# UltronAI/Depth-VO-Feat

Measured on AMD Instinct MI355X. Metric: KITTI 256x832 stereo-seq samples/sec fwd+bwd, higher is better.
Workload: dtype f32

## Files before the change

### depth-vo-feat_amd/csrc/conv_pipe.h

```cpp
#pragma once
#include "dvf_common.h"

namespace dvfp {

#ifdef DVF_TUNING
#define DVF_STAMP(a, var) do { if ((a).stamps) asm volatile("s_memtime %0\n\ts_waitcnt lgkmcnt(0)" : "=s"(var) :: "memory"); } while (0)
#define DVF_STAMP_RT(a, var) do { if ((a).stamps) asm volatile("s_memrealtime %0\n\ts_waitcnt lgkmcnt(0)" : "=s"(var) :: "memory"); } while (0)
#define DVF_STAMPS_ON 1
#else
#define DVF_STAMP(a, var) do { } while (0)
#define DVF_STAMP_RT(a, var) do { } while (0)
#define DVF_STAMPS_ON 0
#endif

typedef float f32x16 __attribute__((ext_vector_type(16)));
typedef __attribute__((address_space(3))) void lds_void_t;

__device__ __forceinline__ __amdgpu_buffer_rsrc_t tensor_rsrc(const void *p) {
    const uint64_t v = reinterpret_cast<uint64_t>(p);
    const unsigned lo = __builtin_amdgcn_readfirstlane((unsigned)v), hi = __builtin_amdgcn_readfirstlane((unsigned)(v >> 32));
    return __builtin_amdgcn_make_buffer_rsrc(reinterpret_cast<void *>(((uint64_t)hi << 32) | lo), 0, 0x7FFFFFF0, 0x00020000);
}
constexpr unsigned OOB = 0x80000000u;
__device__ __forceinline__ float bload(__amdgpu_buffer_rsrc_t r, unsigned voff, unsigned soff) {
// ... 13 lines not shown
    int segC[DVF_MAX_SEGS];
    int nseg;
    const float *wp;
    const float *bias;
    float *out;
    int M, N, IH, IW, OH, OW;
    int OS, IS, ncls;
    PClass cls[4];
    int act;
    float alpha, beta;
    int KS, NCH, out_mode, NG;
    int64_t ws_slice;
    int lsw, lsh, TGX, TGY, BW, BH, BN, tilesX, tilesY;
    int x4;
    int blk;
    int SLmax, PSRmax, NST;
    int dbg;
    unsigned long long *stamps;
    const float *mask;
};

__host__ __device__ inline int pipe_row_stride(int RSu, int SW, int SH, int IS) {
    if (SH == 1 || SW >= 32 || (SW % IS) != 0) return RSu;
    const int mod = 32 / IS, want = (SW / IS) % mod;
    const int padded = RSu + ((want - RSu % mod) + mod) % mod;
    return (padded * 8 <= RSu * 9) ? padded : RSu;
}

struct PipeGeo { int PH, PW, PWH, RS, PSR, NPI, XA; };
__host__ __device__ inline PipeGeo pipe_geo(int BH, int BW, int BN, int IS, int TA, int TB, int SW, int SH, int x4 = 0, int bx = 0) {
// ... 9 lines not shown
            int padded = rs;
            while (((padded * IS) & 31) != ((SW * IS) & 31) && padded < rs + 32) padded += 4;
            if (((padded * IS) & 31) == ((SW * IS) & 31) && padded * 8 <= rs * 9) rs = padded;
        }
        g.RS = rs;
        g.PSR = (BN * g.PH * g.RS + 255) & ~255;
        g.NPI = g.PSR >> 8;
        return g;
    }
    g.RS = pipe_row_stride(IS == 2 ? 2 * g.PWH : g.PW, SW, SH, IS);
    g.PSR = (BN * g.PH * g.RS + 63) & ~63;
    g.NPI = g.PSR >> 6;
    return g;
}

template <int V> struct fvec;
template <> struct fvec<1> { typedef float type; };
template <> struct fvec<2> { typedef float type __attribute__((ext_vector_type(2))); };
template <> struct fvec<4> { typedef float type __attribute__((ext_vector_type(4))); };

constexpr int PIPE_THREADS = 384;
constexpr int PIPE_THREADS_4P = 512;
constexpr int PIPE_MAXNPI = 32;

template <int MT, int NT, int WM, int CKH, int TBU, int BLK = 0>
__global__ __launch_bounds__(PIPE_THREADS_4P) void conv_pipe_kernel(const PipeArgs a) {
    constexpr int CK = 2 * CKH, VW = CKH >= 4 ? 4 : CKH, CPG = CKH / VW, MTW = MT * WM;
    constexpr int UNITF = TBU * MTW * 64 * VW;
    typedef typename fvec<VW>::type avec;
    extern __shared__ __attribute__((aligned(16))) float smem[];
    const int stage_floats = a.SLmax + CK * a.PSRmax;
    const int tid = threadIdx.x, lane = tid & 63, nl = lane & 31, kh = lane >> 5;
    const int wave = __builtin_amdgcn_readfirstlane(tid >> 6);
    const int zper = gridDim.z / a.ncls;
    const int zc = blockIdx.z / zper, zr = blockIdx.z - zc * zper;
    const int ng = zr / a.KS, ks = zr - ng * a.KS;
    const PClass c = a.cls[zc];
    const int tX = blockIdx.x % a.tilesX, tY = blockIdx.x / a.tilesX;
    const int oy0 = tY * a.BH, ox0 = tX * a.BW, n0 = ng * a.BN;
    if (oy0 >= c.OHc || ox0 >= c.OWc) return;
    const int mb = blockIdx.y;
    const int SW = 1 << a.lsw, SH = 1 << a.lsh;
// ... 176 lines not shown
    const int NU = c.NTG * CPG;
    int opy[NT], opx[NT], opn[NT];
    int bj[NT][VW];
    const int pxl = nl & (SW - 1), pyl = (nl >> a.lsw) & (SH - 1), pnl = nl >> (a.lsw + a.lsh);
#pragma unroll
    for (int i = 0; i < NT; ++i) {
        const int q = wn * NT + i, tx = q % a.TGX, tyn = q / a.TGX, ty = tyn % a.TGY, tn = tyn / a.TGY;
        const int SN = 32 >> (a.lsw + a.lsh);
        opy[i] = ty * SH + pyl;
        opx[i] = tx * SW + pxl;
        opn[i] = tn * SN + pnl;
        const int bbase = kh * PSR + (opn[i] * geo.PH + opy[i] * a.IS) * RS + (a.x4 ? geo.XA + opx[i] * a.IS : opx[i]);
#pragma unroll
        for (int j = 0; j < VW; ++j) bj[i][j] = bbase + j * 2 * PSR;
    }
    f32x16 acc[MT][NT];
    f32x16 asum[BLK ? MT : 1][BLK ? NT : 1];
#pragma unroll
    for (int m = 0; m < MT; ++m)
#pragma unroll
        for (int i = 0; i < NT; ++i)
#pragma unroll
            for (int r = 0; r < 16; ++r) {
                acc[m][i][r] = 0.f;
                if constexpr (BLK) asum[m][i][r] = 0.f;
            }

    auto consume = [&](int st, auto isc, auto tbec) {
        constexpr int IS = decltype(isc)::value, TBE = decltype(tbec)::value;
        const float *wl = smem + st * stage_floats;
        const float *patch = wl + a.SLmax;
        const float *ap = wl + (wm * MT) * 64 * VW + lane * VW;
        avec af[2][MT];
        float bf[2][TBE][NT][VW];
        int lta = 0, lcpg = 0, lk = 0;
        auto load_bj = [&](auto bufc, auto jc) {
            constexpr int buf = decltype(bufc)::value, j = decltype(jc)::value;
            const float *prow0 = patch + (lta * RS + lcpg * (2 * VW) * PSR);
#pragma unroll
            for (int i = 0; i < NT; ++i) {
                const float *prow = prow0 + bj[i][j];
// ... 21 lines not shown
        };
        auto advance = [&]() {
            ++lk;
            const bool wrap = (lcpg + 1 == CPG);
            lcpg = wrap ? 0 : lcpg + 1;
            lta += wrap ? 1 : 0;
        };
        auto mma_j = [&](auto bufc, auto tpc, auto uc, auto jc) {
            constexpr int buf = decltype(bufc)::value, tp = decltype(tpc)::value, u = decltype(uc)::value, j = decltype(jc)::value;
#pragma unroll
            for (int m = 0; m < MT; ++m) {
                float av;
                if constexpr (VW == 1) av = af[tp][m]; else av = af[tp][m][j];
#pragma unroll
                for (int i = 0; i < NT; ++i)
                    acc[m][i] = __builtin_amdgcn_mfma_f32_32x32x2f32(av, bf[buf][u][i][j], acc[m][i], 0, 0, 0);
            }
        };
        using B0 = std::integral_constant<int, 0>;
        using B1 = std::integral_constant<int, 1>;
        auto step = [&](auto bufc, auto nbufc, auto pbc, auto uc) {
            constexpr int u = decltype(uc)::value, tp = (decltype(pbc)::value + u) & 1;
            using TP = std::integral_constant<int, tp>;
            mma_j(bufc, TP{}, uc, std::integral_constant<int, 0>{});
            __builtin_amdgcn_sched_barrier(0);
            if constexpr (u + 1 < TBE) load_a(std::integral_constant<int, tp ^ 1>{}, lk - 1, std::integral_constant<int, u + 1>{});
            else load_a(std::integral_constant<int, tp ^ 1>{}, lk, std::integral_constant<int, 0>{});
            if constexpr (u == 0) load_bj(nbufc, std::integral_constant<int, 0>{});
            __builtin_amdgcn_sched_barrier(0);
            if constexpr (VW > 1) {
                mma_j(bufc, TP{}, uc, std::integral_constant<int, 1>{});
// ... 19 lines not shown
            if constexpr (TBE > 4) step(bufc, nbufc, pbc, std::integral_constant<int, 4>{});
            if constexpr (TBE > 5) step(bufc, nbufc, pbc, std::integral_constant<int, 5>{});
            if constexpr (TBE > 6) step(bufc, nbufc, pbc, std::integral_constant<int, 6>{});
            advance();
        };
        load_b(B0{});
        load_a(B0{}, 0, std::integral_constant<int, 0>{});
        advance();
        __builtin_amdgcn_sched_barrier(0);
        for (int k = 0; k < NU; k += 2) {
            unit(B0{}, B1{}, std::integral_constant<int, 0>{});
            if (k + 1 < NU) unit(B1{}, B0{}, std::integral_constant<int, TBE & 1>{});
        }
    };

    unsigned long long t_loop0 = 0, t_loop1 = 0, tb0 = 0, tb1 = 0, w_bar = 0;
    DVF_STAMP(a, t_loop0);
    if (!DVF_DBG(a, 8)) {
        int st = 0, since = 0;
        for (int g = g_begin; g < g_end; ++g) {
            DVF_STAMP(a, tb0);
            __syncthreads();
            DVF_STAMP(a, tb1);
            w_bar += tb1 - tb0;
            if (!DVF_DBG(a, 4)) {
                using TBfull = std::integral_constant<int, TBU>;
                using TBless = std::integral_constant<int, (TBU > 1 ? TBU - 1 : 1)>;
                if (a.IS == 2 && !a.x4) consume(st, std::integral_constant<int, 2>{}, TBfull{});
                else if (TBU > 1 && c.TB == TBU - 1 && !DVF_DBG(a, 64)) consume(st, std::integral_constant<int, 1>{}, TBless{});
                else consume(st, std::integral_constant<int, 1>{}, TBfull{});
            }
            if constexpr (BLK) {
                if (++since == a.blk) {
                    since = 0;
#pragma unroll
                    for (int m = 0; m < MT; ++m)
#pragma unroll
                        for (int i = 0; i < NT; ++i) {
                            asum[m][i] += acc[m][i];
#pragma unroll
                            for (int r = 0; r < 16; ++r) acc[m][i][r] = 0.f;
                        }
                }
            }
            st = (st + 1 == a.NST) ? 0 : st + 1;
        }
    }
    if constexpr (BLK) {
#pragma unroll
        for (int m = 0; m < MT; ++m)
#pragma unroll
            for (int i = 0; i < NT; ++i) acc[m][i] += asum[m][i];
    }

    DVF_STAMP(a, t_loop1);
    auto stamp_out = [&]() {
        if (DVF_STAMPS_ON && a.stamps && wave == 0) {
            unsigned long long t_end = 0, r_end = 0;
            asm volatile("s_waitcnt vmcnt(0)" ::: "memory");
            DVF_STAMP(a, t_end);
            DVF_STAMP_RT(a, r_end);
            if (lane == 0) {
                unsigned long long *o = a.stamps + 8 * lin_block;
                o[0] = t_loop0 - t_entry; o[1] = t_loop1 - t_loop0; o[2] = w_bar; o[3] = t_end - t_loop1; o[4] = r_end - r_entry;
            }
        }
    };
    if DVF_DBG(a, 16) { stamp_out(); return; }
    const int m0 = mb * (32 * MTW) + wm * (32 * MT);
    float *outp = a.out + (a.out_mode == 2 ? (int64_t)ks * a.ws_slice : 0);
    const int64_t HW = (int64_t)a.OH * a.OW;
    if (a.mask && a.out_mode == 0) {
#pragma unroll
        for (int i = 0; i < NT; ++i) {
            const int oy = oy0 + opy[i], ox = ox0 + opx[i], n = n0 + opn[i];
            const int Y = oy * a.OS + c.py, X = ox * a.OS + c.px;
            const bool pok = (oy < c.OHc) && (ox < c.OWc) && (Y < a.OH) && (X < a.OW) && (opn[i] < a.BN) && (n < a.N);
            const int64_t base = ((int64_t)n * a.M + m0 + 4 * kh) * HW + (int64_t)Y * a.OW + X;
            float mk[MT][16];
#pragma unroll
            for (int m = 0; m < MT; ++m)
#pragma unroll
                for (int r = 0; r < 16; ++r) {
                    const int ml = m * 32 + (r & 3) + 8 * (r >> 2);
                    const bool ok = pok && (m0 + 4 * kh + ml < a.M);
                    mk[m][r] = a.mask[ok ? base + (int64_t)ml * HW : 0];
                }
#pragma unroll
            for (int m = 0; m < MT; ++m) {
#pragma unroll
                for (int r = 0; r < 16; ++r) {
                    const int ml = m * 32 + (r & 3) + 8 * (r >> 2);
                    if (pok && m0 + 4 * kh + ml < a.M) {
                        outp[base + (int64_t)ml * HW] = mk[m][r] > 0.f ? acc[m][i][r] : 0.f;
                    }
                }
            }
        }
        stamp_out();
        return;
    }
    const bool full_m = m0 + 32 * MT <= a.M;
    auto store_all = [&](auto modec, auto actc, auto fullc) __attribute__((always_inline)) {
        constexpr int MODE = decltype(modec)::value, ACT = decltype(actc)::value;
        constexpr bool FULL = decltype(fullc)::value;
        float bv[MT][16];
        if constexpr (MODE == 0) {
#pragma unroll
            for (int m = 0; m < MT; ++m)
#pragma unroll
                for (int r = 0; r < 16; ++r) bv[m][r] = bias_lds[wm * (32 * MT) + 4 * kh + m * 32 + (r & 3) + 8 * (r >> 2)];
        }
#pragma unroll
        for (int i = 0; i < NT; ++i) {
            const int oy = oy0 + opy[i], ox = ox0 + opx[i], n = n0 + opn[i];
            const int Y = oy * a.OS + c.py, X = ox * a.OS + c.px;
            const bool pok = (oy < c.OHc) && (ox < c.OWc) && (Y < a.OH) && (X < a.OW) && (opn[i] < a.BN) && (n < a.N);
            float *pbase = outp + ((int64_t)n * a.M + m0 + 4 * kh) * HW + (int64_t)Y * a.OW + X;
            if (pok) {
#pragma unroll
                for (int m = 0; m < MT; ++m) {
#pragma unroll
                    for (int r = 0; r < 16; ++r) {
                        const int ml = m * 32 + (r & 3) + 8 * (r >> 2);
                        if (FULL || m0 + 4 * kh + ml < a.M) {
                            float *op = pbase + (int64_t)ml * HW;
                            const float v = acc[m][i][r];
                            if constexpr (MODE == 0) {
                                const float t = v + bv[m][r];
                                if constexpr (ACT == DVF_ACT_RELU) *op = fmaxf(t, 0.f);
                                else if constexpr (ACT == DVF_ACT_SIGMOID_AFFINE) *op = a.alpha * (1.f / (1.f + expf(-t))) + a.beta;
                                else *op = t;
                            } else if constexpr (MODE == 1) {
                                atomicAdd(op, v);
                            } else {
                                *op = v;
                            }
                        }
                    }
                }
            }
        }
    };
    using std::integral_constant;
    auto by_full = [&](auto modec, auto actc) __attribute__((always_inline)) {
        if (full_m) store_all(modec, actc, std::true_type{});
        else store_all(modec, actc, std::false_type{});
    };
    if (a.out_mode == 2) by_full(integral_constant<int, 2>{}, integral_constant<int, DVF_ACT_NONE>{});
    else if (a.out_mode == 1) by_full(integral_constant<int, 1>{}, integral_constant<int, DVF_ACT_NONE>{});
    else if (a.act == DVF_ACT_RELU) by_full(integral_constant<int, 0>{}, integral_constant<int, DVF_ACT_RELU>{});
    else if (a.act == DVF_ACT_SIGMOID_AFFINE) by_full(integral_constant<int, 0>{}, integral_constant<int, DVF_ACT_SIGMOID_AFFINE>{});
    else by_full(integral_constant<int, 0>{}, integral_constant<int, DVF_ACT_NONE>{});
    stamp_out();
}

template <int MT, int NT, int WM>
int launch_pipe_family(const PipeArgs &a, int CKH, int TBU, dim3 grid, size_t lds, hipStream_t st, int threads);

template <int MT, int NT, int WM, int CKH, int TBU>
constexpr bool pipe_has_blk() {
#ifdef DVF_TUNING
    return true;
#else
    return MT == 2 && NT == 1 && WM == 1 && CKH >= 4 && TBU >= 2 && TBU <= 4;
#endif
}

template <int MT, int NT, int WM, int CKH, int TBU, int BLK>
inline int launch_pipe_blk(const PipeArgs &a, dim3 grid, size_t lds, hipStream_t st, int threads) {
    static bool big_lds = false;
    if (lds > 64 * 1024 && !big_lds) {
        if (hipFuncSetAttribute(reinterpret_cast<const void *>(&conv_pipe_kernel<MT, NT, WM, CKH, TBU, BLK>),
                                hipFuncAttributeMaxDynamicSharedMemorySize, 160 * 1024) != hipSuccess)
            return DVF_ERR_LAUNCH;
        big_lds = true;
    }
    conv_pipe_kernel<MT, NT, WM, CKH, TBU, BLK><<<grid, threads, lds, st>>>(a);
    return hipGetLastError() == hipSuccess ? DVF_OK : DVF_ERR_LAUNCH;
}

template <int MT, int NT, int WM, int CKH, int TBU>
inline int launch_pipe_one(const PipeArgs &a, dim3 grid, size_t lds, hipStream_t st, int threads) {
    if (a.blk) {
        if constexpr (pipe_has_blk<MT, NT, WM, CKH, TBU>()) return launch_pipe_blk<MT, NT, WM, CKH, TBU, 1>(a, grid, lds, st, threads);
        else return DVF_ERR_UNSUPPORTED;
    }
    return launch_pipe_blk<MT, NT, WM, CKH, TBU, 0>(a, grid, lds, st, threads);
}

template <int MT, int NT, int WM, int CKH>
inline int launch_pipe_tbu(const PipeArgs &a, int TBU, dim3 grid, size_t lds, hipStream_t st, int threads) {
    switch (TBU) {
// ... 23 lines not shown
```

### depth-vo-feat_amd/csrc/conv_pipe_host.h

```cpp
#pragma once
#include <string.h>
#include "dvf_common.h"
#include "conv_pipe.h"
#include "conv_op.h"

namespace {

using dvfp::PClass;
using dvfp::PipeArgs;
using dvfp::PipeGeo;
using dvfp::pipe_geo;
using dvfp::PIPE_MAXNPI;

struct alignas(8) PackArgsBody {
    const float *w;
    float *wp;
    int w_mode;
    int Mtot, Rtot, KK, m_base, M;
    int nseg, segC[DVF_MAX_SEGS];
    int ncls, NCH, CK, MB, VW, TBU;
    int TB[4], TA[4];
    int SL[4];
    unsigned wp_off[4];
    signed char tapmap[4][52];
// ... 222 lines not shown
                for (int TGX = 1; TGX * TGN <= ntile; TGX *= 2) {
                    const int TGY = ntile / (TGX * TGN), BW = TGX * SW, BH = TGY * SH;
                    if ((BW - 1) * IS + TBmax > 160) continue;
                    const double cov = (double)cdiv(OWc, BW) * BW * cdiv(OHc, BH) * BH * cdiv(N, BN) * BN;
                    const double narrow = (SW >= 16 ? 0.0 : (SW == 8 ? 0.12 : 0.3)) + (BW >= 32 ? 0.0 : 0.08);
                    const double cost = cov * (1.0 + narrow + 0.02 * lsh + 0.02 * lsn) + 1e-3 * (BW + BH);
                    if (cost < best.cov) best = PipeTiles{lsw, lsh, TGX, TGY, TGN, BN, cost};
                }
            }
        }
    }
    return best;
}


int plan_pipe(const ConvOp &op, PipePlan &pl) {
    if (op.ncls < 1) return DVF_ERR_UNSUPPORTED;
    const ClassSpec *cls = op.cls;
    const int ncls = op.ncls, Tmax = op.Tmax, TAmax = op.TAmax, TBmax = op.TBmax, OHc = op.OHc, OWc = op.OWc;
    const bool head_fwd = op.head_fwd;
    PipeArgs &a = pl.a;
    a = PipeArgs{};
    for (int s = 0; s < op.nseg; ++s) a.segC[s] = op.segC[s];
    a.nseg = op.nseg; a.M = op.M;
    a.N = op.N; a.IH = op.IH; a.IW = op.IW; a.OH = op.OH; a.OW = op.OW;
    a.act = op.act; a.alpha = op.alpha; a.beta = op.beta;
    a.ncls = ncls; a.OS = cls[0].OS; a.IS = cls[0].IS;
    const PipeOverride ov = pipe_override();
    static const int smallm = dvf_tune("DVF_PIPE_SMALLM") ? atoi(dvf_tune("DVF_PIPE_SMALLM")) : 0;
    int ctot = 0;
    for (int s = 0; s < a.nseg; ++s) ctot += a.segC[s];
    static const int headc = dvf_tune("DVF_PIPE_HEADC") ? atoi(dvf_tune("DVF_PIPE_HEADC")) : 128;
    const bool wide_head = head_fwd && a.M <= 4 && ncls == 1 && ctot >= headc && Tmax == 9;
    const bool small_ok = a.M > 16 || wide_head || (!(smallm & 8) && a.M <= 16 && ncls > 1) ||
                          ((smallm & 2) && a.M <= 16) || ((smallm & 4) && a.M > 16);
    if (a.M <= 32 && !ov.on && !small_ok) return DVF_ERR_UNSUPPORTED;
    if (ov.on && ov.KS < 0) return DVF_ERR_UNSUPPORTED;
    int maxc = 0;
    for (int s = 0; s < a.nseg; ++s) maxc = a.segC[s] > maxc ? a.segC[s] : maxc;
    const int64_t px = (int64_t)OHc * OWc;
    int TBU = TBmax;
    if (TBU == 6) TBU = 7;
    if (TBU > 7) return DVF_ERR_UNSUPPORTED;
    int MT = a.M > 32 ? 2 : 1;
    int BN = 1;
    if (px <= 64) { while (BN < a.N && BN * px < 128 && BN < 32) BN *= 2; }
    int WM = 1;
    if (px * BN <= 64 && a.M >= 128) WM = 2;
    int NT = 2;
    if (ov.on) {
        if (ov.MT) MT = ov.MT;
        if (ov.WM) WM = ov.WM;
        if (ov.BN) BN = ov.BN;
    }
    if (WM == 2 || MT == 2) NT = 1;
    const int WN = 4 / WM;
    auto nblocks = [&](const PipeTiles &tp) {
        return (int64_t)cdiv(OWc, tp.TGX << tp.lsw) * cdiv(OHc, tp.TGY << tp.lsh) * cdiv(a.M, 32 * MT * WM) *
               cdiv(a.N, tp.BN) * ncls;
    };
    PipeTiles tp = pipe_tiles(OHc, OWc, a.N, WN * NT, BN, a.IS, TBmax);
    if (tp.cov >= 1e30) return DVF_ERR_UNSUPPORTED;
    int64_t nblk = nblocks(tp);
    if (NT == 2 && nblk < 512 && !(ov.on && ov.NT)) {
        PipeTiles tp1 = pipe_tiles(OHc, OWc, a.N, WN * 1, BN, a.IS, TBmax);
        if (tp1.cov < 1e30) { NT = 1; tp = tp1; nblk = nblocks(tp); }
    }
    if (ov.on && ov.NT && WM == 1 && MT == 1) {
        NT = ov.NT;
        tp = pipe_tiles(OHc, OWc, a.N, WN * NT, BN, a.IS, TBmax);
        if (tp.cov >= 1e30) return DVF_ERR_UNSUPPORTED;
        nblk = nblocks(tp);
    }
    a.lsw = tp.lsw; a.lsh = tp.lsh; a.TGX = tp.TGX; a.TGY = tp.TGY; a.BN = tp.BN;
    a.BW = tp.TGX << tp.lsw; a.BH = tp.TGY << tp.lsh;
    a.tilesX = cdiv(OWc, a.BW); a.tilesY = cdiv(OHc, a.BH); a.NG = cdiv(a.N, a.BN);
    const int SW = 1 << a.lsw, SH = 1 << a.lsh, MB = 32 * MT * WM;
    auto slab = [&](int CK, int TA) { return (TA * TBU * CK * MB + 255) & ~255; };
    static const int ks_thr = dvf_tune("DVF_PIPE_KSTHR") ? atoi(dvf_tune("DVF_PIPE_KSTHR")) : 160;
    static const int ks_tgt = dvf_tune("DVF_PIPE_KSTGT") ? atoi(dvf_tune("DVF_PIPE_KSTGT")) : 256;
    const int KS0 = nblk < ks_thr ? (int)(ks_tgt / nblk) : 1;
    static const int big_lds_kb = dvf_tune("DVF_PIPE_BIGLDS_KB") ? atoi(dvf_tune("DVF_PIPE_BIGLDS_KB")) : 150;
    const size_t PIPE_LDS_BUDGET = (nblk * KS0 <= 256 ? big_lds_kb : 76) * 1024;
    struct Depth { int ok, CK, NST, PSRmax; size_t lds; };
    auto depth_for = [&](int x4) {
        Depth d{0, 0, 3, 0, 0};
        for (int i = 0; i < ncls; ++i) {
            const PipeGeo g = pipe_geo(a.BH, a.BW, a.BN, a.IS, cls[i].TA, TBU, SW, SH, x4, cls[i].bx);
            if (g.NPI > PIPE_MAXNPI) return d;
            d.PSRmax = g.PSR > d.PSRmax ? g.PSR : d.PSRmax;
        }
        auto lds_bytes = [&](int CK) { return ((size_t)d.NST * (slab(CK, TAmax) + (size_t)CK * d.PSRmax) + MB) * 4; };
        int CK = TBU >= 5 ? 8 : 16;
// ... 11 lines not shown
        if (ov.on && ov.NST) d.NST = ov.NST;
        if ((CK != 4 && CK != 8 && CK != 16) || lds_bytes(CK) > 150 * 1024) return d;
        d.ok = 1; d.CK = CK; d.lds = lds_bytes(CK);
        return d;
    };
    int want_x4 = (a.IW % 4 == 0 && (a.BW * a.IS) % 4 == 0) ? 1 : 0;
    if (const char *e = dvf_tune("DVF_PIPE_X4")) want_x4 = want_x4 && atoi(e) != 0;
    const Depth d1 = depth_for(0), d4 = want_x4 ? depth_for(1) : Depth{0, 0, 3, 0, 0};
    static const bool x4_force = dvf_tune("DVF_PIPE_X4") && atoi(dvf_tune("DVF_PIPE_X4")) == 2;
    const bool use4 = d4.ok && (!d1.ok || x4_force || (d4.CK >= d1.CK && d4.NST >= d1.NST));
    const Depth dd = use4 ? d4 : d1;
    if (!dd.ok) return DVF_ERR_UNSUPPORTED;
    a.x4 = use4 ? 1 : 0;
    a.PSRmax = dd.PSRmax;
    const int CK = dd.CK, NST = dd.NST;
    a.NST = NST;
    a.SLmax = slab(CK, TAmax);
    a.NCH = 0;
    for (int s = 0; s < a.nseg; ++s) a.NCH += cdiv(a.segC[s], CK);
    const int mblocks = cdiv(a.M, MB);
    unsigned off = 0;
    for (int i = 0; i < ncls; ++i) {
        const ClassSpec &c = cls[i];
        const int SL = slab(CK, c.TA);
        a.cls[i] = PClass{c.py, c.px, c.by, c.bx, c.TA, c.TB, c.OHc, c.OWc, SL, c.TA, off};
        const int64_t nf = (int64_t)mblocks * a.NCH * SL;
        if ((int64_t)off + nf >= ((int64_t)1 << 29)) return DVF_ERR_UNSUPPORTED;
        off += (unsigned)nf;
    }
    pl.packed_floats = off;
    int KS = KS0;
    if (ov.on && ov.KS) KS = ov.KS;
    if (KS > a.NCH) KS = a.NCH;
    if (KS < 1) KS = 1;
    if ((int64_t)a.NG * KS * ncls > 65535) return DVF_ERR_UNSUPPORTED;
    a.KS = KS;
    pl.ws_floats = (op.covers && KS > 1) ? (int64_t)KS * a.N * a.M * a.OH * a.OW : 0;
    for (int s2 = 0; s2 < a.nseg; ++s2)
        if ((int64_t)a.N * a.segC[s2] * a.IH * a.IW * 4 >= ((int64_t)1 << 31) - 16) return DVF_ERR_UNSUPPORTED;
    pl.MT = MT; pl.NT = NT; pl.WM = WM; pl.CKH = CK / 2; pl.TBU = TBU; pl.lds = dd.lds;
    pl.pack_lds = (size_t)32 * ((CK * op.KK) | 1) * sizeof(float);
    if (pl.pack_lds > 64 * 1024) return DVF_ERR_UNSUPPORTED;
    pl.grid = dim3(a.tilesX * a.tilesY, mblocks, a.NG * KS * ncls);
    {
        const int per_chunk = CK * TAmax * TBmax;
        const int64_t kseq = (int64_t)cdiv(a.NCH, KS) * per_chunk;
        static const int blk_knob = dvf_tune("DVF_PIPE_BLK") ? atoi(dvf_tune("DVF_PIPE_BLK")) : -1;
        static const int blk_terms = dvf_tune("DVF_PIPE_BLKT") ? atoi(dvf_tune("DVF_PIPE_BLKT")) : 0;
        const bool deep = MT == 2 && NT == 1 && WM == 1 && CK >= 8 && TBU >= 2 && TBU <= 4 && kseq >= 512 &&
                          ((int64_t)pl.grid.x * pl.grid.y * pl.grid.z <= 256 || pl.lds > 76 * 1024);
        int every = blk_terms > 0 ? (blk_terms + per_chunk / 2) / per_chunk : 1;
        if (every < 1) every = 1;
        a.blk = blk_knob == 0 ? 0 : blk_knob > 0 ? blk_knob : blk_terms > 0 ? (kseq >= 384 ? every : 0) : (deep ? 1 : 0);
    }
    {
        const int64_t nblocks_total = (int64_t)pl.grid.x * pl.grid.y * pl.grid.z;
        static const bool no4p = dvf_tune("DVF_PIPE_NO4P") != nullptr;
        static const int mt1_4p = dvf_tune("DVF_PIPE_MT1_4P") ? atoi(dvf_tune("DVF_PIPE_MT1_4P")) : 1;
        pl.threads = (!no4p && (pl.lds > 76 * 1024 || nblocks_total <= 256 || (MT == 1 && mt1_4p))) ? dvfp::PIPE_THREADS_4P : dvfp::PIPE_THREADS;
    }
    return DVF_OK;
}

int launch_pipe(const PipeArgs &a, const PipePlan &pl, hipStream_t st) {
    using dvfp::launch_pipe_family;
    if (pl.WM == 2) {
        if (pl.NT != 1) return DVF_ERR_UNSUPPORTED;
        return pl.MT == 2 ? launch_pipe_family<2, 1, 2>(a, pl.CKH, pl.TBU, pl.grid, pl.lds, st, pl.threads)
                          : launch_pipe_family<1, 1, 2>(a, pl.CKH, pl.TBU, pl.grid, pl.lds, st, pl.threads);
    }
    if (pl.WM != 1) return DVF_ERR_UNSUPPORTED;
    if (pl.MT == 2 && pl.NT == 2) return DVF_ERR_UNSUPPORTED;
    if (pl.MT == 2) return launch_pipe_family<2, 1, 1>(a, pl.CKH, pl.TBU, pl.grid, pl.lds, st, pl.threads);
    if (pl.NT == 2) return launch_pipe_family<1, 2, 1>(a, pl.CKH, pl.TBU, pl.grid, pl.lds, st, pl.threads);
    return launch_pipe_family<1, 1, 1>(a, pl.CKH, pl.TBU, pl.grid, pl.lds, st, pl.threads);
}

int run_pipe(const ConvOp &op, const PipePlan &pl, const ConvIO &io, const float *packed, float *ws, int64_t ws_floats,
             hipStream_t st) {
    PipeArgs a = pl.a;
// ... 12 lines not shown
    a.out = out;
    if (mode == 2) { a.out = ws; a.ws_slice = total; }
    if (const char *e = dvf_tune("DVF_DBG")) a.dbg = atoi(e);
    a.stamps = nullptr;
#ifdef DVF_TUNING
    if (dvf_tune("DVF_STAMPS")) {
        const size_t nb = (size_t)pl.grid.x * pl.grid.y * pl.grid.z;
        if (!g_stamp_buf && hipMalloc(&g_stamp_buf, STAMP_MAX_BLOCKS * 64) != hipSuccess) return DVF_ERR_LAUNCH;
        if (nb <= STAMP_MAX_BLOCKS) {
            if (hipMemsetAsync(g_stamp_buf, 0, nb * 64, st) != hipSuccess) return DVF_ERR_LAUNCH;
            a.stamps = g_stamp_buf;
            g_stamp_blocks = (int)nb;
        }
    }
#endif
    dvf_plan_note(DVF_K_PIPE, pl.MT, pl.NT, pl.WM, 2 * pl.CKH, pl.TBU, a.KS, a.BN, a.NST, pl.threads, (int)pl.lds, mode | (a.ncls << 4) | (a.x4 << 8) | ((a.blk ? 1 : 0) << 9));
    if (dvf_tune("DVF_PIPE_DEBUG"))
        fprintf(stderr, "[pipe] M %d chunks %d N %d out %dx%d cls %d | MT %d NT %d WM %d CK %d TBU %d KS %d BN %d tile %dx%d "
                "(sub %dx%d) grid %ux%ux%u lds %zu x%d mode %d\n", a.M, a.NCH, a.N, a.OH, a.OW, a.ncls, pl.MT, pl.NT, pl.WM,
                2 * pl.CKH, pl.TBU, a.KS, a.BN, a.BH, a.BW, 1 << a.lsh, 1 << a.lsw, pl.grid.x, pl.grid.y, pl.grid.z, pl.lds, a.NST, mode);
    int rc = launch_pipe(a, pl, st);
    if (rc) return rc;
    const int64_t nb = (total + 255) / 256;
    if (mode == 2 && a.KS >= 8 && HW < ((int64_t)1 << 30)) {
        splitk_reduce_kpar_kernel<<<(unsigned)((total + 63) / 64), 256, 0, st>>>(ws, out, a.bias, a.mask, a.KS, total, a.M, (int)HW,
                                                                                a.act, a.alpha, a.beta);
        DVF_LAUNCH_CHECK();
    } else if (mode == 2 && a.mask) {
        int chunks = 1;
        const int64_t planes = (int64_t)a.N * a.M;
        while (planes * chunks < 1024 && HW / (chunks * 2) >= 256) chunks *= 2;
// ... 8 lines not shown
        DVF_LAUNCH_CHECK();
    }
    if (mode == 1 && a.mask)
        return dvf_act_bwd(out, a.mask, out, nullptr, a.N, a.M, (int)HW, DVF_ACT_RELU, 1.f, 0.f, 1, nullptr, 0, st);
    return DVF_OK;
}

PackArgs pack_job(const ConvOp &op, const PipePlan &pl, const float *w, float *packed, int *blocks) {
    const PipeArgs &a = pl.a;
    PackArgs p{};
    p.w = w; p.wp = packed; p.w_mode = op.w_mode; p.Mtot = op.Mtot; p.Rtot = op.Rtot; p.KK = op.KK;
    p.m_base = op.m_base; p.M = a.M; p.nseg = a.nseg;
    for (int s = 0; s < a.nseg; ++s) p.segC[s] = a.segC[s];
    p.ncls = op.ncls; p.NCH = a.NCH; p.CK = 2 * pl.CKH; p.MB = 32 * pl.MT * pl.WM; p.VW = pl.CKH >= 4 ? 4 : pl.CKH;
    p.TBU = pl.TBU;
    for (int c = 0; c < op.ncls; ++c) {
        p.SL[c] = a.cls[c].SL;
        p.TB[c] = op.cls[c].TB;
        p.TA[c] = op.cls[c].TA;
        p.wp_off[c] = a.cls[c].wp_off;
        for (int t = 0; t < op.cls[c].TA * op.cls[c].TB; ++t) p.tapmap[c][t] = (signed char)op.cls[c].tapmap[t];
    }
    *blocks = a.NCH * cdiv(a.M, p.MB) * (p.MB >> 5);
    return p;
}

int launch_pack(const ConvOp &op, const PipePlan &pl, const float *w, float *packed, hipStream_t st) {
    int blocks;
    const PackArgs p = pack_job(op, pl, w, packed, &blocks);
    conv_pack_kernel<<<dim3(p.NCH, blocks / p.NCH), 256, pl.pack_lds, st>>>(p);
// ... 6 lines not shown
```

Before: 614.7.

## Fuse four stride-2 transposed-conv parity classes into one shared-patch kernel

Adds a fused path for stride-2 transposed/upsampling convolutions with 3x3 to 5x5 kernels. It computes all four output parity classes in one block from a single staged input patch, keeping four accumulator sets and a compile-time schedule of tap products. Previously each class was a separate grid slice that re-staged its own patch. This cuts redundant patch loads and launches, at the cost of four times the accumulator registers, MT and NT forced to 1, and a new packed-weight tap order.

```diff
diff --git a/depth-vo-feat_amd/csrc/conv_pipe.h b/depth-vo-feat_amd/csrc/conv_pipe.h
--- a/depth-vo-feat_amd/csrc/conv_pipe.h
+++ b/depth-vo-feat_amd/csrc/conv_pipe.h
@@ -1,4 +1,5 @@
 #pragma once
+#include <utility>
 #include "dvf_common.h"
 
 namespace dvfp {
@@ -51,6 +52,7 @@
     int lsw, lsh, TGX, TGY, BW, BH, BN, tilesX, tilesY;
     int x4;
     int blk;
+    int fused;
     int SLmax, PSRmax, NST;
     int dbg;
     unsigned long long *stamps;
@@ -90,6 +92,53 @@
     return g;
 }
 
+struct FusedAxis { int n[2], base[2], amax[2], TU, UB; };
+__host__ __device__ constexpr int fused_pad(int K) { return K == 5 ? 2 : 1; }
+__host__ __device__ constexpr FusedAxis fused_axis(int K) {
+    FusedAxis f{};
+    for (int c = 0; c < 2; ++c) {
+        int amax = -1;
+        for (int t = K - 1; t >= 0; --t)
+            if ((c + fused_pad(K) - t) % 2 == 0) { amax = t; break; }
+        f.amax[c] = amax; f.n[c] = amax / 2 + 1; f.base[c] = (c + fused_pad(K) - amax) / 2;
+    }
+    f.UB = f.base[0] < f.base[1] ? f.base[0] : f.base[1];
+    const int e0 = f.base[0] + f.n[0], e1 = f.base[1] + f.n[1];
+    f.TU = (e0 > e1 ? e0 : e1) - f.UB;
+    return f;
+}
+__host__ __device__ constexpr int fused_tap(int K, int c, int r) {
+    const FusedAxis f = fused_axis(K);
+    const int i = r - (f.base[c] - f.UB);
+    return (i >= 0 && i < f.n[c]) ? i : -1;
+}
+struct FusedProd { int rb, q; };
+__host__ __device__ constexpr FusedProd fused_prod(int K, int ra, int k, int *count = nullptr) {
+    const int TU = fused_axis(K).TU;
+    FusedProd out{-1, -1};
+    int cnt = 0;
+    for (int rb = 0; rb < TU; ++rb)
+        for (int cy = 0; cy < 2; ++cy)
+            for (int cx = 0; cx < 2; ++cx)
+                if (fused_tap(K, cy, ra) >= 0 && fused_tap(K, cx, rb) >= 0) {
+                    if (cnt == k) out = FusedProd{rb, cy * 2 + cx};
+                    ++cnt;
+                }
+    if (count) *count = cnt;
+    return out;
+}
+__host__ __device__ constexpr int fused_row_count(int K, int ra) { int n = 0; fused_prod(K, ra, -1, &n); return n; }
+__host__ __device__ constexpr int fused_row_start(int K, int ra) {
+    int s = 0;
+    for (int r = 0; r < ra; ++r) s += fused_row_count(K, r);
+    return s;
+}
+
+template <class F, int... I>
+__device__ __forceinline__ void static_for_seq(F &&f, std::integer_sequence<int, I...>) { (f(std::integral_constant<int, I>{}), ...); }
+template <int N, class F>
+__device__ __forceinline__ void static_for(F &&f) { static_for_seq(f, std::make_integer_sequence<int, N>{}); }
+
 template <int V> struct fvec;
 template <> struct fvec<1> { typedef float type; };
 template <> struct fvec<2> { typedef float type __attribute__((ext_vector_type(2))); };
@@ -99,9 +148,10 @@
 constexpr int PIPE_THREADS_4P = 512;
 constexpr int PIPE_MAXNPI = 32;
 
-template <int MT, int NT, int WM, int CKH, int TBU, int BLK = 0>
+template <int MT, int NT, int WM, int CKH, int TBU, int BLK = 0, int FUSED = 0>
 __global__ __launch_bounds__(PIPE_THREADS_4P) void conv_pipe_kernel(const PipeArgs a) {
     constexpr int CK = 2 * CKH, VW = CKH >= 4 ? 4 : CKH, CPG = CKH / VW, MTW = MT * WM;
+    constexpr int NC = FUSED ? 4 : 1;
     constexpr int UNITF = TBU * MTW * 64 * VW;
     typedef typename fvec<VW>::type avec;
     extern __shared__ __attribute__((aligned(16))) float smem[];
@@ -308,17 +358,19 @@
 #pragma unroll
         for (int j = 0; j < VW; ++j) bj[i][j] = bbase + j * 2 * PSR;
     }
-    f32x16 acc[MT][NT];
-    f32x16 asum[BLK ? MT : 1][BLK ? NT : 1];
-#pragma unroll
-    for (int m = 0; m < MT; ++m)
-#pragma unroll
-        for (int i = 0; i < NT; ++i)
-#pragma unroll
-            for (int r = 0; r < 16; ++r) {
-                acc[m][i][r] = 0.f;
-                if constexpr (BLK) asum[m][i][r] = 0.f;
-            }
+    f32x16 acc[NC][MT][NT];
+    f32x16 asum[BLK ? NC : 1][BLK ? MT : 1][BLK ? NT : 1];
+#pragma unroll
+    for (int q = 0; q < NC; ++q)
+#pragma unroll
+        for (int m = 0; m < MT; ++m)
+#pragma unroll
+            for (int i = 0; i < NT; ++i)
+#pragma unroll
+                for (int r = 0; r < 16; ++r) {
+                    acc[q][m][i][r] = 0.f;
+                    if constexpr (BLK) asum[q][m][i][r] = 0.f;
+                }
 
     auto consume = [&](int st, auto isc, auto tbec) {
         constexpr int IS = decltype(isc)::value, TBE = decltype(tbec)::value;
@@ -370,7 +422,7 @@
                 if constexpr (VW == 1) av = af[tp][m]; else av = af[tp][m][j];
 #pragma unroll
                 for (int i = 0; i < NT; ++i)
-                    acc[m][i] = __builtin_amdgcn_mfma_f32_32x32x2f32(av, bf[buf][u][i][j], acc[m][i], 0, 0, 0);
+                    acc[0][m][i] = __builtin_amdgcn_mfma_f32_32x32x2f32(av, bf[buf][u][i][j], acc[0][m][i], 0, 0, 0);
             }
         };
         using B0 = std::integral_constant<int, 0>;
@@ -420,6 +472,58 @@
         }
     };
 
+    auto consume_fused = [&](int st, auto kfc) {
+        constexpr int KF = decltype(kfc)::value, TU = fused_axis(KF).TU, NPROD = KF * KF, NUN = CPG * TU;
+        static_assert(TU == TBU, "a fused instantiation stages TU columns");
+        const float *wl = smem + st * stage_floats;
+        const float *patch = wl + a.SLmax;
+        const float *ap = wl + (wm * MT) * 64 * VW + lane * VW;
+        avec af[2][MT];
+        float bf[2][TU][NT][VW];
+        auto load_bj = [&](auto bufc, auto unc, auto jc) {
+            constexpr int buf = decltype(bufc)::value, un = decltype(unc)::value, j = decltype(jc)::value;
+            const float *prow0 = patch + ((un % TU) * RS + (un / TU) * (2 * VW) * PSR);
+#pragma unroll
+            for (int i = 0; i < NT; ++i) {
+                const float *prow = prow0 + bj[i][j];
+#pragma unroll
+                for (int u = 0; u < TU; ++u) bf[buf][u][i][j] = prow[u];
+            }
+        };
+        auto load_a = [&](auto tpc, auto gpc) {
+            constexpr int tp = decltype(tpc)::value, gp = decltype(gpc)::value;
+#pragma unroll
+            for (int m = 0; m < MT; ++m) af[tp][m] = *reinterpret_cast<const avec *>(ap + (gp * MTW + m) * 64 * VW);
+        };
+        using std::integral_constant;
+        static_for<VW>([&](auto jc) { load_bj(integral_constant<int, 0>{}, integral_constant<int, 0>{}, jc); });
+        load_a(integral_constant<int, 0>{}, integral_constant<int, 0>{});
+        __builtin_amdgcn_sched_barrier(0);
+        static_for<NUN>([&](auto unc) {
+            constexpr int un = decltype(unc)::value, ra = un % TU, buf = un & 1;
+            constexpr int start = (un / TU) * NPROD + fused_row_start(KF, ra);
+            static_for<fused_row_count(KF, ra)>([&](auto kc) {
+                constexpr int k = decltype(kc)::value, gp = start + k, tp = gp & 1;
+                constexpr int rb = fused_prod(KF, ra, k).rb, q = fused_prod(KF, ra, k).q;
+                static_for<VW>([&](auto jc) {
+                    constexpr int j = decltype(jc)::value;
+#pragma unroll
+                    for (int m = 0; m < MT; ++m) {
+                        float av;
+                        if constexpr (VW == 1) av = af[tp][m]; else av = af[tp][m][j];
+#pragma unroll
+                        for (int i = 0; i < NT; ++i)
+                            acc[q][m][i] = __builtin_amdgcn_mfma_f32_32x32x2f32(av, bf[buf][rb][i][j], acc[q][m][i], 0, 0, 0);
+                    }
+                    __builtin_amdgcn_sched_barrier(0);
+                    if constexpr (j == 0 && gp + 1 < CPG * NPROD) load_a(integral_constant<int, tp ^ 1>{}, integral_constant<int, gp + 1>{});
+                    if constexpr (k == 0 && un + 1 < NUN) load_bj(integral_constant<int, buf ^ 1>{}, integral_constant<int, un + 1>{}, jc);
+                    __builtin_amdgcn_sched_barrier(0);
+                });
+            });
+        });
+    };
+
     unsigned long long t_loop0 = 0, t_loop1 = 0, tb0 = 0, tb1 = 0, w_bar = 0;
     DVF_STAMP(a, t_loop0);
     if (!DVF_DBG(a, 8)) {
@@ -432,7 +536,8 @@
             if (!DVF_DBG(a, 4)) {
                 using TBfull = std::integral_constant<int, TBU>;
                 using TBless = std::integral_constant<int, (TBU > 1 ? TBU - 1 : 1)>;
-                if (a.IS == 2 && !a.x4) consume(st, std::integral_constant<int, 2>{}, TBfull{});
+                if constexpr (FUSED) consume_fused(st, std::integral_constant<int, FUSED>{});
+                else if (a.IS == 2 && !a.x4) consume(st, std::integral_constant<int, 2>{}, TBfull{});
                 else if (TBU > 1 && c.TB == TBU - 1 && !DVF_DBG(a, 64)) consume(st, std::integral_constant<int, 1>{}, TBless{});
                 else consume(st, std::integral_constant<int, 1>{}, TBfull{});
             }
@@ -440,13 +545,15 @@
                 if (++since == a.blk) {
                     since = 0;
 #pragma unroll
-                    for (int m = 0; m < MT; ++m)
-#pragma unroll
-                        for (int i = 0; i < NT; ++i) {
-                            asum[m][i] += acc[m][i];
-#pragma unroll
-                            for (int r = 0; r < 16; ++r) acc[m][i][r] = 0.f;
-                        }
+                    for (int q = 0; q < NC; ++q)
+#pragma unroll
+                        for (int m = 0; m < MT; ++m)
+#pragma unroll
+                            for (int i = 0; i < NT; ++i) {
+                                asum[q][m][i] += acc[q][m][i];
+#pragma unroll
+                                for (int r = 0; r < 16; ++r) acc[q][m][i][r] = 0.f;
+                            }
                 }
             }
             st = (st + 1 == a.NST) ? 0 : st + 1;
@@ -454,9 +561,11 @@
     }
     if constexpr (BLK) {
 #pragma unroll
-        for (int m = 0; m < MT; ++m)
-#pragma unroll
-            for (int i = 0; i < NT; ++i) acc[m][i] += asum[m][i];
+        for (int q = 0; q < NC; ++q)
+#pragma unroll
+            for (int m = 0; m < MT; ++m)
+#pragma unroll
+                for (int i = 0; i < NT; ++i) acc[q][m][i] += asum[q][m][i];
     }
 
     DVF_STAMP(a, t_loop1);
@@ -477,10 +586,12 @@
     float *outp = a.out + (a.out_mode == 2 ? (int64_t)ks * a.ws_slice : 0);
     const int64_t HW = (int64_t)a.OH * a.OW;
     if (a.mask && a.out_mode == 0) {
+        static_for<NC>([&](auto qc) {
+        constexpr int q = decltype(qc)::value;
 #pragma unroll
         for (int i = 0; i < NT; ++i) {
             const int oy = oy0 + opy[i], ox = ox0 + opx[i], n = n0 + opn[i];
-            const int Y = oy * a.OS + c.py, X = ox * a.OS + c.px;
+            const int Y = oy * a.OS + (FUSED ? (q >> 1) : c.py), X = ox * a.OS + (FUSED ? (q & 1) : c.px);
             const bool pok = (oy < c.OHc) && (ox < c.OWc) && (Y < a.OH) && (X < a.OW) && (opn[i] < a.BN) && (n < a.N);
             const int64_t base = ((int64_t)n * a.M + m0 + 4 * kh) * HW + (int64_t)Y * a.OW + X;
             float mk[MT][16];
@@ -498,11 +609,12 @@
                 for (int r = 0; r < 16; ++r) {
                     const int ml = m * 32 + (r & 3) + 8 * (r >> 2);
                     if (pok && m0 + 4 * kh + ml < a.M) {
-                        outp[base + (int64_t)ml * HW] = mk[m][r] > 0.f ? acc[m][i][r] : 0.f;
+                        outp[base + (int64_t)ml * HW] = mk[m][r] > 0.f ? acc[q][m][i][r] : 0.f;
                     }
                 }
             }
         }
+        });
         stamp_out();
         return;
     }
@@ -517,10 +629,12 @@
 #pragma unroll
                 for (int r = 0; r < 16; ++r) bv[m][r] = bias_lds[wm * (32 * MT) + 4 * kh + m * 32 + (r & 3) + 8 * (r >> 2)];
         }
+        static_for<NC>([&](auto qc) {
+        constexpr int q = decltype(qc)::value;
 #pragma unroll
         for (int i = 0; i < NT; ++i) {
             const int oy = oy0 + opy[i], ox = ox0 + opx[i], n = n0 + opn[i];
-            const int Y = oy * a.OS + c.py, X = ox * a.OS + c.px;
+            const int Y = oy * a.OS + (FUSED ? (q >> 1) : c.py), X = ox * a.OS + (FUSED ? (q & 1) : c.px);
             const bool pok = (oy < c.OHc) && (ox < c.OWc) && (Y < a.OH) && (X < a.OW) && (opn[i] < a.BN) && (n < a.N);
             float *pbase = outp + ((int64_t)n * a.M + m0 + 4 * kh) * HW + (int64_t)Y * a.OW + X;
             if (pok) {
@@ -531,7 +645,7 @@
                         const int ml = m * 32 + (r & 3) + 8 * (r >> 2);
                         if (FULL || m0 + 4 * kh + ml < a.M) {
                             float *op = pbase + (int64_t)ml * HW;
-                            const float v = acc[m][i][r];
+                            const float v = acc[q][m][i][r];
                             if constexpr (MODE == 0) {
                                 const float t = v + bv[m][r];
                                 if constexpr (ACT == DVF_ACT_RELU) *op = fmaxf(t, 0.f);
@@ -547,6 +661,7 @@
                 }
             }
         }
+        });
     };
     using std::integral_constant;
     auto by_full = [&](auto modec, auto actc) __attribute__((always_inline)) {
@@ -563,6 +678,7 @@
 
 template <int MT, int NT, int WM>
 int launch_pipe_family(const PipeArgs &a, int CKH, int TBU, dim3 grid, size_t lds, hipStream_t st, int threads);
+int launch_pipe_fused(const PipeArgs &a, int WM, int CKH, dim3 grid, size_t lds, hipStream_t st, int threads);
 
 template <int MT, int NT, int WM, int CKH, int TBU>
 constexpr bool pipe_has_blk() {
@@ -573,16 +689,16 @@
 #endif
 }
 
-template <int MT, int NT, int WM, int CKH, int TBU, int BLK>
+template <int MT, int NT, int WM, int CKH, int TBU, int BLK, int FUSED = 0>
 inline int launch_pipe_blk(const PipeArgs &a, dim3 grid, size_t lds, hipStream_t st, int threads) {
     static bool big_lds = false;
     if (lds > 64 * 1024 && !big_lds) {
-        if (hipFuncSetAttribute(reinterpret_cast<const void *>(&conv_pipe_kernel<MT, NT, WM, CKH, TBU, BLK>),
+        if (hipFuncSetAttribute(reinterpret_cast<const void *>(&conv_pipe_kernel<MT, NT, WM, CKH, TBU, BLK, FUSED>),
                                 hipFuncAttributeMaxDynamicSharedMemorySize, 160 * 1024) != hipSuccess)
             return DVF_ERR_LAUNCH;
         big_lds = true;
     }
-    conv_pipe_kernel<MT, NT, WM, CKH, TBU, BLK><<<grid, threads, lds, st>>>(a);
+    conv_pipe_kernel<MT, NT, WM, CKH, TBU, BLK, FUSED><<<grid, threads, lds, st>>>(a);
     return hipGetLastError() == hipSuccess ? DVF_OK : DVF_ERR_LAUNCH;
 }
 
diff --git a/depth-vo-feat_amd/csrc/conv_pipe_host.h b/depth-vo-feat_amd/csrc/conv_pipe_host.h
--- a/depth-vo-feat_amd/csrc/conv_pipe_host.h
+++ b/depth-vo-feat_amd/csrc/conv_pipe_host.h
@@ -260,8 +260,33 @@
 }
 
 
-int plan_pipe(const ConvOp &op, PipePlan &pl) {
-    if (op.ncls < 1) return DVF_ERR_UNSUPPORTED;
+int fused_kernel_size(const ConvOp &op) {
+    if (op.ncls != 4 || !op.covers) return 0;
+    int K = 0;
+    for (int k = 3; k <= 5; ++k)
+        if (op.KK == k * k) K = k;
+    if (!K) return 0;
+    const dvfp::FusedAxis f = dvfp::fused_axis(K);
+    for (int i = 0; i < 4; ++i) {
+        const ClassSpec &c = op.cls[i];
+        if (c.OS != 2 || c.IS != 1 || c.py < 0 || c.py > 1 || c.px < 0 || c.px > 1) return 0;
+        if (c.TA != f.n[c.py] || c.TB != f.n[c.px] || c.by != f.base[c.py] || c.bx != f.base[c.px]) return 0;
+        for (int ta = 0; ta < c.TA; ++ta)
+            for (int tb = 0; tb < c.TB; ++tb)
+                if (c.tapmap[ta * c.TB + tb] != (f.amax[c.py] - 2 * ta) * K + f.amax[c.px] - 2 * tb) return 0;
+    }
+    return K;
+}
+
+int plan_pipe_form(const ConvOp &op_in, PipePlan &pl, int fusedK) {
+    ConvOp op = op_in;
+    if (fusedK) {
+        const dvfp::FusedAxis f = dvfp::fused_axis(fusedK);
+        const int nmax = f.n[0] > f.n[1] ? f.n[0] : f.n[1];
+        op.ncls = 1;
+        op.cls[0] = ClassSpec{2, 0, 0, 1, f.UB, f.UB, f.TU, f.TU, op_in.OHc, op_in.OWc, {0}};
+        op.Tmax = nmax * nmax; op.TAmax = op.TBmax = f.TU;
+    }
     const ClassSpec *cls = op.cls;
     const int ncls = op.ncls, Tmax = op.Tmax, TAmax = op.TAmax, TBmax = op.TBmax, OHc = op.OHc, OWc = op.OWc;
     const bool head_fwd = op.head_fwd;
@@ -279,7 +304,7 @@
     static const int headc = dvf_tune("DVF_PIPE_HEADC") ? atoi(dvf_tune("DVF_PIPE_HEADC")) : 128;
     const bool wide_head = head_fwd && a.M <= 4 && ncls == 1 && ctot >= headc && Tmax == 9;
     const bool small_ok = a.M > 16 || wide_head || (!(smallm & 8) && a.M <= 16 && ncls > 1) ||
-                          ((smallm & 2) && a.M <= 16) || ((smallm & 4) && a.M > 16);
+                          ((smallm & 2) && a.M <= 16) || ((smallm & 4) && a.M > 16) || fusedK;
     if (a.M <= 32 && !ov.on && !small_ok) return DVF_ERR_UNSUPPORTED;
     if (ov.on && ov.KS < 0) return DVF_ERR_UNSUPPORTED;
     int maxc = 0;
@@ -299,7 +324,8 @@
         if (ov.WM) WM = ov.WM;
         if (ov.BN) BN = ov.BN;
     }
-    if (WM == 2 || MT == 2) NT = 1;
+    if (fusedK) MT = 1;
+    if (WM == 2 || MT == 2 || fusedK) NT = 1;
     const int WN = 4 / WM;
     auto nblocks = [&](const PipeTiles &tp) {
         return (int64_t)cdiv(OWc, tp.TGX << tp.lsw) * cdiv(OHc, tp.TGY << tp.lsh) * cdiv(a.M, 32 * MT * WM) *
@@ -312,7 +338,7 @@
         PipeTiles tp1 = pipe_tiles(OHc, OWc, a.N, WN * 1, BN, a.IS, TBmax);
         if (tp1.cov < 1e30) { NT = 1; tp = tp1; nblk = nblocks(tp); }
     }
-    if (ov.on && ov.NT && WM == 1 && MT == 1) {
+    if (ov.on && ov.NT && WM == 1 && MT == 1 && !fusedK) {
         NT = ov.NT;
         tp = pipe_tiles(OHc, OWc, a.N, WN * NT, BN, a.IS, TBmax);
         if (tp.cov >= 1e30) return DVF_ERR_UNSUPPORTED;
@@ -322,7 +348,7 @@
     a.BW = tp.TGX << tp.lsw; a.BH = tp.TGY << tp.lsh;
     a.tilesX = cdiv(OWc, a.BW); a.tilesY = cdiv(OHc, a.BH); a.NG = cdiv(a.N, a.BN);
     const int SW = 1 << a.lsw, SH = 1 << a.lsh, MB = 32 * MT * WM;
-    auto slab = [&](int CK, int TA) { return (TA * TBU * CK * MB + 255) & ~255; };
+    auto slab = [&](int CK, int TA) { return ((fusedK ? op.KK : TA * TBU) * CK * MB + 255) & ~255; };
     static const int ks_thr = dvf_tune("DVF_PIPE_KSTHR") ? atoi(dvf_tune("DVF_PIPE_KSTHR")) : 160;
     static const int ks_tgt = dvf_tune("DVF_PIPE_KSTGT") ? atoi(dvf_tune("DVF_PIPE_KSTGT")) : 256;
     const int KS0 = nblk < ks_thr ? (int)(ks_tgt / nblk) : 1;
@@ -364,6 +390,8 @@
     a.x4 = use4 ? 1 : 0;
     a.PSRmax = dd.PSRmax;
     const int CK = dd.CK, NST = dd.NST;
+    if (fusedK && CK < 8) return DVF_ERR_UNSUPPORTED;
+    a.fused = fusedK;
     a.NST = NST;
     a.SLmax = slab(CK, TAmax);
     a.NCH = 0;
@@ -393,11 +421,11 @@
     if (pl.pack_lds > 64 * 1024) return DVF_ERR_UNSUPPORTED;
     pl.grid = dim3(a.tilesX * a.tilesY, mblocks, a.NG * KS * ncls);
     {
-        const int per_chunk = CK * TAmax * TBmax;
+        const int per_chunk = CK * (fusedK ? Tmax : TAmax * TBmax);
         const int64_t kseq = (int64_t)cdiv(a.NCH, KS) * per_chunk;
         static const int blk_knob = dvf_tune("DVF_PIPE_BLK") ? atoi(dvf_tune("DVF_PIPE_BLK")) : -1;
         static const int blk_terms = dvf_tune("DVF_PIPE_BLKT") ? atoi(dvf_tune("DVF_PIPE_BLKT")) : 0;
-        const bool deep = MT == 2 && NT == 1 && WM == 1 && CK >= 8 && TBU >= 2 && TBU <= 4 && kseq >= 512 &&
+        const bool deep = (fusedK ? a.M > 32 : MT == 2) && NT == 1 && WM == 1 && CK >= 8 && TBU >= 2 && TBU <= 4 && kseq >= 512 &&
                           ((int64_t)pl.grid.x * pl.grid.y * pl.grid.z <= 256 || pl.lds > 76 * 1024);
         int every = blk_terms > 0 ? (blk_terms + per_chunk / 2) / per_chunk : 1;
         if (every < 1) every = 1;
@@ -412,8 +440,24 @@
     return DVF_OK;
 }
 
+bool fused_wanted(const ConvOp &op, int K) {
+    if (const char *e = dvf_tune("DVF_PIPE_FUSED")) return atoi(e) != 0;
+    return true;
+}
+
+int plan_pipe(const ConvOp &op, PipePlan &pl) {
+    if (op.ncls < 1) return DVF_ERR_UNSUPPORTED;
+    const int K = fused_kernel_size(op);
+    if (K && fused_wanted(op, K) && plan_pipe_form(op, pl, K) == DVF_OK) return DVF_OK;
+    return plan_pipe_form(op, pl, 0);
+}
+
 int launch_pipe(const PipeArgs &a, const PipePlan &pl, hipStream_t st) {
     using dvfp::launch_pipe_family;
+    if (a.fused) {
+        if (pl.MT != 1 || pl.NT != 1) return DVF_ERR_UNSUPPORTED;
+        return dvfp::launch_pipe_fused(a, pl.WM, pl.CKH, pl.grid, pl.lds, st, pl.threads);
+    }
     if (pl.WM == 2) {
         if (pl.NT != 1) return DVF_ERR_UNSUPPORTED;
         return pl.MT == 2 ? launch_pipe_family<2, 1, 2>(a, pl.CKH, pl.TBU, pl.grid, pl.lds, st, pl.threads)
@@ -456,7 +500,7 @@
         }
     }
 #endif
-    dvf_plan_note(DVF_K_PIPE, pl.MT, pl.NT, pl.WM, 2 * pl.CKH, pl.TBU, a.KS, a.BN, a.NST, pl.threads, (int)pl.lds, mode | (a.ncls << 4) | (a.x4 << 8) | ((a.blk ? 1 : 0) << 9));
+    dvf_plan_note(DVF_K_PIPE, pl.MT, pl.NT, pl.WM, 2 * pl.CKH, pl.TBU, a.KS, a.BN, a.NST, pl.threads, (int)pl.lds, mode | ((a.fused ? 4 : a.ncls) << 4) | (a.x4 << 8) | ((a.blk ? 1 : 0) << 9) | ((a.fused ? 1 : 0) << 10));
     if (dvf_tune("DVF_PIPE_DEBUG"))
         fprintf(stderr, "[pipe] M %d chunks %d N %d out %dx%d cls %d | MT %d NT %d WM %d CK %d TBU %d KS %d BN %d tile %dx%d "
                 "(sub %dx%d) grid %ux%ux%u lds %zu x%d mode %d\n", a.M, a.NCH, a.N, a.OH, a.OW, a.ncls, pl.MT, pl.NT, pl.WM,
@@ -495,6 +539,21 @@
     for (int s = 0; s < a.nseg; ++s) p.segC[s] = a.segC[s];
     p.ncls = op.ncls; p.NCH = a.NCH; p.CK = 2 * pl.CKH; p.MB = 32 * pl.MT * pl.WM; p.VW = pl.CKH >= 4 ? 4 : pl.CKH;
     p.TBU = pl.TBU;
+    if (a.fused) {
+        const int K = a.fused;
+        const dvfp::FusedAxis f = dvfp::fused_axis(K);
+        p.ncls = 1; p.TBU = op.KK; p.TB[0] = op.KK; p.TA[0] = 1; p.SL[0] = a.cls[0].SL; p.wp_off[0] = 0;
+        int np = 0;
+        for (int ra = 0; ra < f.TU; ++ra)
+            for (int k = 0; k < dvfp::fused_row_count(K, ra); ++k) {
+                const dvfp::FusedProd pr = dvfp::fused_prod(K, ra, k);
+                const int cy = pr.q >> 1, cx = pr.q & 1;
+                p.tapmap[0][np++] = (signed char)((f.amax[cy] - 2 * dvfp::fused_tap(K, cy, ra)) * K +
+                                                  f.amax[cx] - 2 * dvfp::fused_tap(K, cx, pr.rb));
+            }
+        *blocks = a.NCH * cdiv(a.M, p.MB) * (p.MB >> 5);
+        return p;
+    }
     for (int c = 0; c < op.ncls; ++c) {
         p.SL[c] = a.cls[c].SL;
         p.TB[c] = op.cls[c].TB;
diff --git a/depth-vo-feat_amd/csrc/conv_pipe_inst_f.hip b/depth-vo-feat_amd/csrc/conv_pipe_inst_f.hip
--- /dev/null
+++ b/depth-vo-feat_amd/csrc/conv_pipe_inst_f.hip
@@ -0,0 +1,32 @@
+#include "conv_pipe.h"
+namespace dvfp {
+namespace {
+
+template <int WM, int CKH, int K>
+int launch_fused_one(const PipeArgs &a, dim3 grid, size_t lds, hipStream_t st, int threads) {
+    constexpr int TU = fused_axis(K).TU;
+    if (a.blk) return launch_pipe_blk<1, 1, WM, CKH, TU, 1, K>(a, grid, lds, st, threads);
+    return launch_pipe_blk<1, 1, WM, CKH, TU, 0, K>(a, grid, lds, st, threads);
+}
+
+template <int WM, int CKH>
+int launch_fused_k(const PipeArgs &a, dim3 grid, size_t lds, hipStream_t st, int threads) {
+    switch (a.fused) {
+        case 3: return launch_fused_one<WM, CKH, 3>(a, grid, lds, st, threads);
+        case 4: return launch_fused_one<WM, CKH, 4>(a, grid, lds, st, threads);
+        case 5: return launch_fused_one<WM, CKH, 5>(a, grid, lds, st, threads);
+        default: return DVF_ERR_UNSUPPORTED;
+    }
+}
+
+}
+
+int launch_pipe_fused(const PipeArgs &a, int WM, int CKH, dim3 grid, size_t lds, hipStream_t st, int threads) {
+    if (WM == 1 && CKH == 4) return launch_fused_k<1, 4>(a, grid, lds, st, threads);
+    if (WM == 1 && CKH == 8) return launch_fused_k<1, 8>(a, grid, lds, st, threads);
+    if (WM == 2 && CKH == 4) return launch_fused_k<2, 4>(a, grid, lds, st, threads);
+    if (WM == 2 && CKH == 8) return launch_fused_k<2, 8>(a, grid, lds, st, threads);
+    return DVF_ERR_UNSUPPORTED;
+}
+
+}
```

After: 619.8 (median of 6 runs). About the same (+0.8%).
